# poja/Cattus

Measured on AMD Instinct MI355X. Metric: MCTS node-evals/sec (chess 20x256 net, batch 256), higher is better.
Workload: dtype f16x2

## Files before the change

### cattus_amd/csrc/evaluator.hip

```cpp
#include <hip/hip_runtime.h>

#include <algorithm>
#include <atomic>
#include <chrono>
#include <condition_variable>
#include <cmath>
#include <cstdarg>
#include <cstdio>
#include <cstdlib>
#include <cstring>
#include <deque>
#include <functional>
#include <map>
#include <memory>
#include <mutex>
#include <new>
#include <shared_mutex>
#include <string>
#include <thread>
#include <vector>

#include <dlfcn.h>

#include "../../include/cattus_hip.h"
// ... 112 lines not shown
            return CATTUS_OK;
        }
        hipError_t e = hipMalloc(&p, bytes ? bytes : 16);
        if (e != hipSuccess) return fail(CATTUS_E_NOMEM, "hipMalloc(%zu) failed: %s", bytes, hipGetErrorString(e));
        return CATTUS_OK;
    }
    int upload(const void* src, size_t bytes, DevArena* arena = nullptr) {
        int rc = alloc(bytes, arena);
        if (rc) return rc;
        HIP_TRY(hipMemcpy(p, src, bytes, hipMemcpyHostToDevice));
        return CATTUS_OK;
    }
    template <typename T>
    T* as() const {
        return reinterpret_cast<T*>(p);
    }
};

struct PinnedBuf {
    void* p = nullptr;
    ~PinnedBuf() {
        if (p) (void)hipHostFree(p);
    }
    int alloc(size_t bytes) {
        hipError_t e = hipHostMalloc(&p, bytes ? bytes : 16, hipHostMallocDefault);
        if (e != hipSuccess) return fail(CATTUS_E_NOMEM, "hipHostMalloc(%zu) failed: %s", bytes, hipGetErrorString(e));
        return CATTUS_OK;
    }
    template <typename T>
    T* as() const {
        return reinterpret_cast<T*>(p);
    }
};

std::shared_mutex g_pin_mu;
std::map<const char*, size_t> g_pinned;
struct Roctx {
    int (*push)(const char*) = nullptr;
    int (*pop)() = nullptr;
    Roctx() {
        const char* on = getenv("CATTUS_ROCTX");
        if (!on || on[0] != '1') return;
        for (const char* name : {"librocprofiler-sdk-roctx.so", "libroctx64.so"}) {
            if (void* h = dlopen(name, RTLD_NOW | RTLD_GLOBAL)) {
                push = reinterpret_cast<int (*)(const char*)>(dlsym(h, "roctxRangePushA"));
                pop = reinterpret_cast<int (*)()>(dlsym(h, "roctxRangePop"));
                if (push && pop) return;
                push = nullptr, pop = nullptr;
// ... 28 lines not shown
}

struct ConvLayer {
    DevBuf w, b;
    DevBuf wf;
    DevBuf wu, bw;
    uint32_t cin = 0;
};

struct ServerBatch {
    uint64_t seq = 0;
    uint32_t count = 0, collected = 0;
    bool sealed = false, running = false, done = false;
    int status = CATTUS_OK;
    std::string error;
    std::chrono::steady_clock::time_point t0;
    std::vector<uint64_t> planes;
    std::vector<float> policy, value;
    std::vector<uint8_t> taken;
};

constexpr int NLANES = CATTUS_HIP_LANES;

struct Lane {
    hipStream_t stream = nullptr;
    hipEvent_t done = nullptr;
    DevBuf d_planes, x0, a, t, y, hv, h1, d_policy, d_value;
    DevBuf d_legal_idx, d_legal_cnt, d_probs;
    uint32_t legal_stride = 0;
    PinnedBuf h_planes, h_policy, h_value;
    DevBuf tower_layers, tower_ready;
    PinnedBuf h_tower_err;
    uint32_t tower_nlayers = 0;
    std::mutex mu;
    ~Lane() {
        if (done) (void)hipEventDestroy(done);
        if (stream) (void)hipStreamDestroy(stream);
    }
};

}

struct cattus_eval {
    DevArena arena;
    cattus_net_desc d{};
    cattus_eval_config cfg{};
    bool tuned = false;
    bool simple = false;
    DevBuf d1w, d1b, d2w, d2b, svw, svb, spw, spb;
    bool wait_spin = true;
    Act act = Act::F32;
    uint32_t hw = 0, bpad = 0, cpad0 = 0;
    uint32_t slots = 64;
    uint32_t fpad = 0;
    bool tower64 = false;
    bool resident_tower = true;
    DevBuf t64_layers;
    bool tower64s = false;
    DevBuf t64s_bias;
    bool t64s_fuse_heads = true;
// ... 6 lines not shown
    bool wino_persist = true;
    std::atomic<bool> persist_ok{true};
    uint32_t persist_spin = 1u << 18;
    uint32_t cus = 0;
    bool wino_inplace = true;
    bool split_wfrag = true;
    bool stream_shift_on = true;
    int stream_shift = 0;
    ConvOpts conv_opts;
    DevBuf d_saturated;
    bool t64_layer_steps = true;
    int device = 0;

    ConvLayer stem;
    std::vector<std::unique_ptr<ConvLayer>> c1, c2;
    DevBuf head_w, head_b, w1t, b1, w2, b2, wpt, bp;
    uint32_t kvp = 0, kpp = 0;

    Lane lanes[NLANES];
    std::atomic<unsigned> lane_rr{0};

    std::mutex stat_mu;
    cattus_stats stats{};
    uint64_t stats_tower_fallbacks = 0;

    std::mutex srv_mu;
    std::condition_variable srv_cv, done_cv;
    std::deque<std::unique_ptr<ServerBatch>> batches;
    uint64_t next_seq = 1;
    bool flush_req = false, stop = false;
    std::thread servers[NLANES];

    ~cattus_eval() {
        {
            std::lock_guard<std::mutex> lk(srv_mu);
            stop = true;
        }
        srv_cv.notify_all();
        done_cv.notify_all();
        for (auto& t : servers)
            if (t.joinable()) t.join();
    }
};

namespace {

size_t blob_floats(const cattus_net_desc& d) {
    const size_t hw = (size_t)d.board * d.board, F = d.filters;
    if (F == 0) {
        const size_t K = (size_t)d.planes * hw;
        return 2 * (K * K + K) + K + 1 + (size_t)d.moves * K + d.moves;
    }
    size_t n = F * d.planes * 9 + 4 * F;
    n += (size_t)d.blocks * (2 * F * F * 9 + 6 * F);
    n += (size_t)d.vhc * F + 2 * (size_t)d.vhc + (size_t)FC_HIDDEN * d.vhc * hw + FC_HIDDEN + FC_HIDDEN + 1;
    n += (size_t)d.phc * F + 2 * (size_t)d.phc + (size_t)d.moves * d.phc * hw + d.moves;
    return n;
}

bool wino_shape_ok(const cattus_eval* e, uint32_t cin, uint32_t cout) {
    return e->wino_k4 ? wino4_supported(e->bpad, cin, cout, e->d.board) : wino_supported(e->bpad, cin, cout, e->d.board);
}

std::mutex g_chain_mu;
hipEvent_t g_chain[64] = {};
int chain_persistent_launch(int device, hipStream_t st, const std::function<void()>& launch) {
    std::lock_guard<std::mutex> lk(g_chain_mu);
    hipEvent_t& ev = g_chain[device & 63];
    if (!ev) {
        HIP_TRY(hipEventCreateWithFlags(&ev, hipEventDisableTiming));
    } else {
        HIP_TRY(hipStreamWaitEvent(st, ev, 0));
    }
    launch();
    HIP_TRY(hipEventRecord(ev, st));
    return CATTUS_OK;
}

int upload_conv(cattus_eval* e, ConvLayer& L, const Folded& f, uint32_t cout, uint32_t cin, uint32_t cout_pad, uint32_t cin_pad) {
    int rc;
    if (!e->tuned) {
        L.cin = cin;
        if ((rc = L.b.upload(f.b.data(), cout * sizeof(float)))) return rc;
        return L.w.upload(f.w.data(), f.w.size() * sizeof(float));
    }
    L.cin = cin_pad;
    if (e->act == Act::F16S) {
        std::vector<float> b((size_t)2 * cout_pad, 0.0f);
        memcpy(b.data(), f.b.data(), cout * sizeof(float));
        std::vector<_Float16> w((size_t)9 * cout_pad * 2 * cin_pad, (_Float16)0.0f);
        for (uint32_t co = 0; co < cout_pad; co++) {
            float m = 0.0f;
            if (co < cout)
                for (uint32_t t = 0; t < 9; t++)
                    for (uint32_t ci = 0; ci < cin; ci++) m = std::max(m, fabsf(f.w[((size_t)t * cout + co) * cin + ci]));
            int sh = 0;
            if (m > 0.0f && std::isfinite(m)) sh = std::min(100, std::max(-100, 10 - ilogbf(m)));
            b[cout_pad + co] = ldexpf(1.0f, -sh);
            if (co >= cout) continue;
// ... 270 lines not shown
        HIP_TRY(hipEventCreateWithFlags(&L.done, hipEventBlockingSync | hipEventDisableTiming));
        if ((rc = L.d_planes.alloc(B * d.planes * e->cfg.plane_words * 8))) return rc;
        if ((rc = L.x0.alloc(bp_ * slots * e->cpad0 * esz))) return rc;
        if ((rc = L.a.alloc(bp_ * slots * FA * esz, &e->arena))) return rc;
        if ((rc = L.t.alloc(bp_ * slots * FA * esz, &e->arena))) return rc;
        if ((rc = L.y.alloc(bp_ * slots * FA * esz, e->wino_inplace ? nullptr : &e->arena))) return rc;
        const size_t hv_bytes = (size_t)(e->tuned ? (bp_ + 31) / 32 * 32 : bp_) * (e->kvp + e->kpp) * hesz;
        if ((rc = L.hv.alloc(hv_bytes))) return rc;
        HIP_TRY(hipMemset(L.hv.p, 0, hv_bytes));
        if ((rc = L.h1.alloc(bp_ * FC_HIDDEN * 4))) return rc;
        if ((rc = L.d_policy.alloc(B * d.moves * 4))) return rc;
        if ((rc = L.d_value.alloc(B * 4))) return rc;
        if ((rc = L.h_planes.alloc(B * d.planes * e->cfg.plane_words * 8))) return rc;
        if ((rc = L.h_policy.alloc(B * d.moves * 4))) return rc;
        if ((rc = L.h_value.alloc(B * 4))) return rc;
        if (e->tuned && e->act == Act::F16S && e->wino_k4 && e->wino_persist && e->wino_inplace && d.blocks > 0 && e->c1[0]->wu.p) {
            std::vector<Wino4TowerLayer> tl;
            for (uint32_t i = 0; i < d.blocks; i++) {
                tl.push_back(Wino4TowerLayer{L.a.as<float>(), e->c1[i]->wu.p, e->c1[i]->bw.as<float>(), nullptr, L.t.as<float>()});
                tl.push_back(Wino4TowerLayer{L.t.as<float>(), e->c2[i]->wu.p, e->c2[i]->bw.as<float>(), L.a.as<float>(), L.a.as<float>()});
            }
            L.tower_nlayers = (uint32_t)tl.size();
            if ((rc = L.tower_layers.upload(tl.data(), tl.size() * sizeof(Wino4TowerLayer)))) return rc;
            if ((rc = L.tower_ready.alloc(64 + (size_t)tl.size() * (bp_ / 4) * 4))) return rc;
            if ((rc = L.h_tower_err.alloc(4))) return rc;
            *L.h_tower_err.as<unsigned>() = 0;
        }
    }
    return CATTUS_OK;
}

struct TowerTimer {
    std::vector<hipEvent_t> ev;
    size_t used = 0;
};

int enqueue_forward(cattus_eval* e, Lane& L, const uint64_t* d_planes, uint32_t n, float* d_policy, float* d_value,
                    hipStream_t st, TowerTimer* tt = nullptr) {
    const cattus_net_desc& d = e->d;
    const uint32_t F = d.filters, hw = e->hw, S = d.board, w64 = e->cfg.plane_words;
    auto ev = [&](bool stop) -> hipEvent_t {
        if (!tt || tt->used >= tt->ev.size()) return nullptr;
        (void)stop;
        return tt->ev[tt->used++];
    };
    void *a = L.a.p, *t = L.t.p, *y = L.y.p;
    uint32_t nb = n;
    if (e->simple) {
        const uint32_t K = d.planes * hw;
// ... 36 lines not shown
            launch_tower64_split(ta, nb * e->slots, e->t64s_depth, st, s0, s1);
        } else {
            const bool fused_stem = d.planes <= 32 && e->cpad0 == (uint32_t)act_kc(e->act) && !e->pack_separately;
            const StemInput stem_in{d_planes, n, d.planes, w64};
            if (!fused_stem) launch_pack_planes_nhwc(e->act, d_planes, n, nb, d.planes, w64, S, e->cpad0, L.x0.p, st);
            hipEvent_t s0 = ev(false), s1 = ev(true);
            const int last_flags = act_f16_family(e->act) ? CONV_OUT_F32 : 0;
            const bool wfrag = e->act == Act::F16S && e->split_wfrag;
            const int wflag = wfrag ? CONV_W_FRAG : 0;
            auto wptr = [&](const ConvLayer& c) { return wfrag ? c.wf.p : c.w.p; };
            launch_conv3x3_mfma(e->act, L.x0.p, wptr(e->stem), e->stem.b.as<float>(), nullptr, a, nb, e->cpad0, FP, S, st, s0, s1,
                                fused_stem ? &stem_in : nullptr,
                                wflag | (d.blocks == 0 ? last_flags : e->act == Act::F16S && e->c1[0]->wu.p ? CONV_OUT_F32 | CONV_WINO_IN : 0), e->conv_opts);
            const bool wino = d.blocks > 0 && e->c1[0]->wu.p != nullptr;
            auto conv = [&](const ConvLayer& c, const void* in, const void* res, void* out, int lflags) {
                hipEvent_t s0 = ev(false), s1 = ev(true);
                if (wino && e->wino_k8) launch_conv3x3_wino8((const float*)in, c.wu.p, c.bw.as<float>(), (const float*)res, (float*)out, nb, FP, FP, st, s0, s1, e->conv_opts.saturated);
                else if (wino && e->wino_k4) launch_conv3x3_wino4((const float*)in, c.wu.p, c.bw.as<float>(), (const float*)res, (float*)out, nb, FP, FP, st, s0, s1, e->conv_opts.saturated);
                else if (wino) launch_conv3x3_wino((const float*)in, c.wu.p, c.bw.as<float>(), (const float*)res, (float*)out, nb, FP, FP, st, s0, s1, e->conv_opts.saturated);
                else launch_conv3x3_mfma(e->act, in, wptr(c), c.b.as<float>(), res, out, nb, FP, FP, S, st, s0, s1, nullptr, wflag | lflags, e->conv_opts);
            };
            if (wino && !e->wino_k8 && L.tower_nlayers && e->persist_ok.load(std::memory_order_relaxed) && wino4_tower_fits(nb, FP, e->cus)) {
                hipEvent_t s0 = ev(false), s1 = ev(true);
                unsigned* const tower_err = L.tower_ready.as<unsigned>();
                HIP_TRY(hipMemsetAsync(L.tower_ready.p, 0, 64 + (size_t)L.tower_nlayers * (nb / 4) * 4, st));
                int crc = chain_persistent_launch(e->device, st, [&] {
                    launch_tower_wino4(L.tower_layers.as<Wino4TowerLayer>(), L.tower_nlayers, tower_err + 16, tower_err,
                                       e->conv_opts.saturated, nb, FP, e->persist_spin, e->cus, st, s0, s1);
                });
                if (crc) return crc;
                HIP_TRY(hipMemcpyAsync(L.h_tower_err.p, tower_err, 4, hipMemcpyDeviceToHost, st));
            } else
            for (uint32_t i = 0; i < d.blocks; i++) {
                conv(*e->c1[i], a, nullptr, t, 0);
                if (wino && e->wino_inplace) {
                    conv(*e->c2[i], t, a, a, 0);
                    continue;
                }
                conv(*e->c2[i], t, a, y, i + 1 == d.blocks ? last_flags : 0);
                std::swap(a, y);
            }
        }
    } else {
        launch_planes_to_tensor_nchw(d_planes, n, d.planes, w64, S, n, L.x0.as<float>(), st);
        hipEvent_t s0 = ev(false), s1 = ev(true);
        launch_conv3x3_generic(L.x0.as<float>(), e->stem.w.as<float>(), e->stem.b.as<float>(), nullptr, (float*)a, n,
                               d.planes, F, S, st, s0, s1);
        for (uint32_t i = 0; i < d.blocks; i++) {
            s0 = ev(false), s1 = ev(true);
            launch_conv3x3_generic((float*)a, e->c1[i]->w.as<float>(), e->c1[i]->b.as<float>(), nullptr, (float*)t, n, F,
                                   F, S, st, s0, s1);
            s0 = ev(false), s1 = ev(true);
            launch_conv3x3_generic((float*)t, e->c2[i]->w.as<float>(), e->c2[i]->b.as<float>(), (float*)a, (float*)y, n,
                                   F, F, S, st, s0, s1);
// ... 4 lines not shown
    if (e->tuned) {
        HeadsMfma hd{};
        hd.conv_w = e->head_w.p, hd.conv_b = e->head_b.as<float>(), hd.hv = L.hv.p;
        hd.w1 = e->w1t.p, hd.b1 = e->b1.as<float>(), hd.h1 = L.h1.as<float>();
        hd.wp = e->wpt.p, hd.bp = e->bp.as<float>(), hd.policy = d_policy;
        hd.hw = hw, hd.vhc = d.vhc, hd.phc = d.phc, hd.kvp = e->kvp, hd.kpp = e->kpp, hd.M = d.moves;
        hd.w2 = e->w2.as<float>(), hd.b2 = e->b2.as<float>(), hd.value = d_value;
        hd.slots = e->slots;
        hd.hv_leaves = (e->bpad + 31) / 32 * 32;
        launch_heads_mfma(head_act(e->act), e->tower64 || (e->tower64s && e->t64s_fuse_heads) ? nullptr : a, n, e->fpad, hd, st);
    } else {
        TowerView tv;
        tv.x = a, tv.act = Act::F32, tv.sb = F * hw, tv.sk = hw, tv.sp = 1;
        launch_head_conv1x1(tv, e->head_w.as<float>(), e->head_b.as<float>(), n, F, d.vhc + d.phc, hw, L.hv.as<float>(), st);
        launch_value_fc1(L.hv.as<float>(), kv + kp, e->w1t.as<float>(), e->b1.as<float>(), n, kv, L.h1.as<float>(), st);
        launch_value_fc2_tanh(L.h1.as<float>(), e->w2.as<float>(), e->b2.as<float>(), n, d_value, st);
        launch_policy_fc(L.hv.as<float>(), kv + kp, kv, e->wpt.as<float>(), e->bp.as<float>(), n, kp, d.moves, d_policy, st);
    }
    hipError_t err = hipGetLastError();
    if (err != hipSuccess) return fail(CATTUS_E_DEVICE, "kernel launch failed: %s", hipGetErrorString(err));
    return CATTUS_OK;
}

void account(cattus_eval* e, uint32_t n, double seconds) {
    std::lock_guard<std::mutex> lk(e->stat_mu);
    cattus_stats& s = e->stats;
    s.run_seconds_ema = 0.01 * s.run_seconds_ema + 0.99 * seconds;
    s.run_seconds_total += seconds;
    s.batches += 1;
    s.positions += n;
    if (n == e->cfg.max_batch) s.full_batches += 1;
}

struct LegalArgs {
    const uint16_t* idx;
    const uint16_t* cnt;
    uint32_t stride;
    float* probs;
};

int eval_host(cattus_eval* e, const uint64_t* planes, uint32_t n, float* policy, float* value, const LegalArgs* lg = nullptr) {
    const cattus_net_desc& d = e->d;
    std::unique_lock<std::mutex> lk;
    Lane* lane = nullptr;
    for (Lane& cand : e->lanes) {
        std::unique_lock<std::mutex> tl(cand.mu, std::try_to_lock);
// ... 34 lines not shown
                                     lg->stride, n, L.d_probs.as<float>(), L.stream))
                return fail(CATTUS_E_INVALID, "legal stride %u exceeds 1024", lg->stride);
            HIP_TRY(hipMemcpyAsync(lg->probs, L.d_probs.p, (size_t)n * lg->stride * 4, hipMemcpyDeviceToHost, L.stream));
        } else {
            HIP_TRY(hipMemcpyAsync(direct ? (void*)policy : L.h_policy.p, L.d_policy.p, (size_t)n * d.moves * 4, hipMemcpyDeviceToHost, L.stream));
        }
        HIP_TRY(hipMemcpyAsync(direct ? (void*)value : L.h_value.p, L.d_value.p, (size_t)n * 4, hipMemcpyDeviceToHost, L.stream));
        return CATTUS_OK;
    };
    auto run_batch = [&]() -> int {
        int rc = enqueue_forward(e, L, L.d_planes.as<uint64_t>(), n, L.d_policy.as<float>(), L.d_value.as<float>(), L.stream);
        if (rc) return rc;
        if ((rc = copy_out())) return rc;
        if (e->wait_spin) {
            HIP_TRY(hipStreamSynchronize(L.stream));
        } else {
            HIP_TRY(hipEventRecord(L.done, L.stream));
            HIP_TRY(hipEventSynchronize(L.done));
        }
        return CATTUS_OK;
    };
    int rc = run_batch();
    if (rc) return rc;
    if (L.h_tower_err.p && *L.h_tower_err.as<volatile unsigned>() != 0) {
        *L.h_tower_err.as<volatile unsigned>() = 0;
        e->persist_ok.store(false, std::memory_order_relaxed);
        {
            std::lock_guard<std::mutex> sl(e->stat_mu);
            e->stats_tower_fallbacks += 1;
        }
        if ((rc = run_batch())) return rc;
    }
    if (!direct) {
        if (!lg) memcpy(policy, L.h_policy.p, (size_t)n * d.moves * 4);
        memcpy(value, L.h_value.p, (size_t)n * 4);
    }
    account(e, n, std::chrono::duration<double>(std::chrono::steady_clock::now() - t0).count());
    return CATTUS_OK;
}

ServerBatch* new_batch(cattus_eval* e) {
    auto b = std::make_unique<ServerBatch>();
    b->seq = e->next_seq++;
    b->planes.resize((size_t)e->cfg.max_batch * e->d.planes * e->cfg.plane_words);
    e->batches.push_back(std::move(b));
    return e->batches.back().get();
}

void server_loop(cattus_eval* e) {
    std::unique_lock<std::mutex> lk(e->srv_mu);
    for (;;) {
        ServerBatch* run = nullptr;
        for (auto& b : e->batches)
// ... 20 lines not shown
            e->srv_cv.wait(lk);
            continue;
        }
        run->running = true;
        const uint32_t n = run->count;
        run->policy.resize((size_t)n * e->d.moves);
        run->value.resize(n);
        run->taken.assign(n, 0);
        lk.unlock();
        const int rc = eval_host(e, run->planes.data(), n, run->policy.data(), run->value.data());
        std::string err = rc ? g_last_error : std::string();
        lk.lock();
        run->status = rc;
        run->error = err;
        run->done = true;
        e->done_cv.notify_all();
    }
}

}


CATTUS_API const char* cattus_hip_last_error(void) { return g_last_error.c_str(); }
CATTUS_API const char* cattus_hip_version(void) { return "cattus_hip 0.2 (gfx950)"; }
CATTUS_API const char* cattus_hip_runtime_note(void) { return g_runtime_note.c_str(); }

CATTUS_API const char* cattus_hip_tower_kernel(const cattus_eval* e) {
    if (!e) return "";
    if (e->simple) return "policy_fc_kernel";
    if (!e->tuned) return "conv3x3_generic_kernel";
    if (e->tower64) return "tower64_lds_kernel";
    if (e->tower64s) return "tower64_split_kernel";
    if (e->act == Act::F16S) return e->d.blocks > 0 && e->c1[0]->wu.p ? (e->wino_k8 ? "conv3x3_wino8_kernel" : e->wino_k4 ? (e->lanes[0].tower_nlayers && e->persist_ok.load() && wino4_tower_fits(e->bpad, e->fpad, e->cus) ? "tower_wino4_kernel" : "conv3x3_wino4_kernel") : "conv3x3_wino_kernel") : e->split_wfrag ? "conv3x3_splitw_kernel" : "conv3x3_split_kernel";
    return "conv3x3_mfma_v2_kernel";
}

CATTUS_API int cattus_hip_stream_shift(const cattus_eval* e) { return e ? e->stream_shift : 0; }

namespace {

struct Switches {
    std::map<std::string, std::string> kv;
    int parse(const char* text) {
        if (!text) return CATTUS_OK;
        static const char* const known[] = {"CATTUS_CONV_CB", "CATTUS_CONV_PBW", "CATTUS_FUSED_STEM", "CATTUS_T64_CH", "CATTUS_T64_LS", "CATTUS_SPLIT_W",
                                            "CATTUS_T64S_HEADS", "CATTUS_T64S_SHAPE", "CATTUS_TOWER64", "CATTUS_FORCE_GENERIC", "CATTUS_WINO_INPLACE",
                                            "CATTUS_ARENA", "CATTUS_WINO_KERNEL", "CATTUS_WINO_PERSIST", "CATTUS_WINO_SPIN", "CATTUS_STREAM_SHIFT"};
// ... 207 lines not shown
    for (uint32_t i = 0; i < n; i++) {
        if (legal_count[i] > legal_stride) return fail(CATTUS_E_INVALID, "leaf %u: %u legal moves > stride %u", i, legal_count[i], legal_stride);
        for (uint32_t k = 0; k < legal_count[i]; k++)
            if (legal_idx[(size_t)i * legal_stride + k] >= e->d.moves)
                return fail(CATTUS_E_INVALID, "leaf %u: policy index %u >= %u", i, legal_idx[(size_t)i * legal_stride + k], e->d.moves);
    }
    const LegalArgs lg{legal_idx, legal_count, legal_stride, probs};
    return eval_host(e, planes, n, nullptr, value, &lg);
}

CATTUS_API int cattus_hip_eval_device(cattus_eval* e, const uint64_t* d_planes, uint32_t n, float* d_policy, float* d_value,
                                      void* stream) {
    return cattus_hip_eval_device_lane(e, 0, d_planes, n, d_policy, d_value, stream);
}

CATTUS_API int cattus_hip_eval_device_lane(cattus_eval* e, uint32_t lane, const uint64_t* d_planes, uint32_t n, float* d_policy,
                                           float* d_value, void* stream) {
    if (!e || !d_planes || !d_policy || !d_value) return fail(CATTUS_E_INVALID, "NULL argument");
    if (n < 1 || n > e->cfg.max_batch) return fail(CATTUS_E_INVALID, "invalid sample len %u, 1..=%u", n, e->cfg.max_batch);
    if (lane >= NLANES) return fail(CATTUS_E_INVALID, "lane %u out of range (%d lanes)", lane, NLANES);
    Lane& L = e->lanes[lane];
    std::lock_guard<std::mutex> lk(L.mu);
    HIP_TRY(hipSetDevice(e->device));
    if (L.h_tower_err.p && *L.h_tower_err.as<volatile unsigned>() != 0) {
        *L.h_tower_err.as<volatile unsigned>() = 0;
        e->persist_ok.store(false, std::memory_order_relaxed);
        return fail(CATTUS_E_DEVICE, "an earlier batch on lane %u ran the tower as one launch and a hand-off wait in it gave up (the device was shared): that batch's "
                                     "outputs are invalid; this evaluator uses the per-layer launches from now on", lane);
    }
    hipStream_t st = (hipStream_t)stream;
    int rc = enqueue_forward(e, L, d_planes, n, d_policy, d_value, st);
    if (rc) return rc;
    std::lock_guard<std::mutex> sl(e->stat_mu);
    e->stats.batches += 1;
    e->stats.positions += n;
    if (n == e->cfg.max_batch) e->stats.full_batches += 1;
    return CATTUS_OK;
}

CATTUS_API int cattus_hip_lane_stream(cattus_eval* e, uint32_t lane, void** stream) {
    if (!e || !stream) return fail(CATTUS_E_INVALID, "NULL argument");
    if (lane >= NLANES) return fail(CATTUS_E_INVALID, "lane %u out of range (%d lanes)", lane, NLANES);
    *stream = (void*)e->lanes[lane].stream;
    return CATTUS_OK;
}

CATTUS_API int cattus_hip_submit(cattus_eval* e, const uint64_t* planes_one, uint64_t* ticket) {
    if (!e || !planes_one || !ticket) return fail(CATTUS_E_INVALID, "NULL argument");
    const size_t words = (size_t)e->d.planes * e->cfg.plane_words;
    std::unique_lock<std::mutex> lk(e->srv_mu);
    if (e->stop) return fail(CATTUS_E_STATE, "evaluator is shutting down");
// ... 111 lines not shown
CATTUS_API int cattus_hip_time_tower(cattus_eval* e, uint32_t n, uint32_t reps, float* avg_launch_us, uint32_t* launches) {
    if (!e || !avg_launch_us || !launches) return fail(CATTUS_E_INVALID, "NULL argument");
    if (n < 1 || n > e->cfg.max_batch || reps < 1) return fail(CATTUS_E_INVALID, "bad n/reps");
    if (e->simple) return fail(CATTUS_E_UNSUPPORTED, "a SimpleTwoHeadedModel has no conv tower to time");
    Lane& L = e->lanes[0];
    std::lock_guard<std::mutex> lk(L.mu);
    HIP_TRY(hipSetDevice(e->device));
    const uint32_t per_fwd = e->tower64 || e->tower64s ? 1 : 1 + 2 * e->d.blocks;
    TowerTimer tt;
    tt.ev.resize((size_t)2 * per_fwd);
    for (auto& ev : tt.ev) HIP_TRY(hipEventCreate(&ev));
    HIP_TRY(hipMemsetAsync(L.d_planes.p, 0x5a, (size_t)n * e->d.planes * e->cfg.plane_words * 8, L.stream));
    double total_ms = 0;
    int rc = CATTUS_OK;
    for (uint32_t rep = 0; rep < reps + 1 && rc == CATTUS_OK; rep++) {
        tt.used = 0;
        rc = enqueue_forward(e, L, L.d_planes.as<uint64_t>(), n, L.d_policy.as<float>(), L.d_value.as<float>(), L.stream, &tt);
        if (rc) break;
        hipError_t err = hipStreamSynchronize(L.stream);
        if (err != hipSuccess) {
            rc = fail(CATTUS_E_DEVICE, "hipStreamSynchronize: %s", hipGetErrorString(err));
            break;
        }
        if (rep == 0) continue;
        for (size_t i = 0; i + 1 < tt.used; i += 2) {
            float ms = 0;
            (void)hipEventElapsedTime(&ms, tt.ev[i], tt.ev[i + 1]);
            total_ms += ms;
        }
    }
    for (auto& ev : tt.ev) (void)hipEventDestroy(ev);
    if (rc) return rc;
    *launches = per_fwd;
    *avg_launch_us = (float)(total_ms * 1000.0 / ((double)reps * per_fwd));
    return CATTUS_OK;
}

CATTUS_API int cattus_hip_mfma_sustained(cattus_eval* e, double seconds, double* tflops) {
    if (!e || !tflops) return fail(CATTUS_E_INVALID, "NULL argument");
    if (!(seconds > 0) || seconds > 30) return fail(CATTUS_E_INVALID, "seconds out of range");
    Lane& L = e->lanes[0];
    std::lock_guard<std::mutex> lk(L.mu);
    HIP_TRY(hipSetDevice(e->device));
    hipDeviceProp_t prop;
    HIP_TRY(hipGetDeviceProperties(&prop, e->device));
    const int cus = prop.multiProcessorCount;
// ... 60 lines not shown
```

### cattus_amd/csrc/kernels.h

```cpp
#pragma once
#include <hip/hip_runtime.h>
#include <stdint.h>

namespace cattus {

inline uint32_t tower_slots(uint32_t S) { return S <= 8 ? 64u : 128u; }
constexpr int ROWS_PER_WG = 256;
constexpr int COUT_PER_WG = 64;

enum class Act : int { F32 = 0, BF16 = 1, F16S = 2, F16 = 3 };

inline bool act_two_bytes(Act a) { return a == Act::BF16 || a == Act::F16; }
inline int act_bytes(Act a) { return act_two_bytes(a) ? 2 : 4; }
inline int act_kc(Act a) { return act_two_bytes(a) ? 64 : 32; }
inline Act head_act(Act a) { return a == Act::BF16 ? Act::BF16 : Act::F32; }
inline bool act_f16_family(Act a) { return a == Act::F16S || a == Act::F16; }

hipError_t prepare_device();

void launch_pack_planes_nhwc(Act act, const uint64_t* planes, uint32_t n, uint32_t bpad, uint32_t C,
                             uint32_t w64, uint32_t S, uint32_t cpad, void* out, hipStream_t st);
void launch_planes_to_tensor_nchw(const uint64_t* planes, uint32_t n, uint32_t C, uint32_t w64, uint32_t S,
                                  uint32_t batch, float* out, hipStream_t st);

// ... 24 lines not shown
    const uint32_t nst = cin_pad / 16 * 16, stage = (ci >> 4) * 16 + f, lane = ((ci >> 3) & 1) * 32 + (co & 31);
    return ((((size_t)(co >> 5) * nst + stage) * 2 + part) * 64 + lane) * 8 + (ci & 7);
}
void launch_conv3x3_wino(const float* in, const void* wu, const float* bias, const float* res, float* out, uint32_t bpad, uint32_t cin,
                         uint32_t cout, hipStream_t st, hipEvent_t ev_start, hipEvent_t ev_stop, unsigned* sat);
hipError_t prepare_wino();

bool wino4_supported(uint32_t bpad, uint32_t cin, uint32_t cout, uint32_t S);
void launch_conv3x3_wino4(const float* in, const void* wu, const float* bias, const float* res, float* out, uint32_t bpad, uint32_t cin,
                          uint32_t cout, hipStream_t st, hipEvent_t ev_start, hipEvent_t ev_stop, unsigned* sat);
hipError_t prepare_wino4();
bool wino8_supported(uint32_t bpad, uint32_t cin, uint32_t cout, uint32_t S);
void launch_conv3x3_wino8(const float* in, const void* wu, const float* bias, const float* res, float* out, uint32_t bpad, uint32_t cin,
                          uint32_t cout, hipStream_t st, hipEvent_t ev_start, hipEvent_t ev_stop, unsigned* sat);
hipError_t prepare_wino8();
struct Wino4TowerLayer {
    const float* in;
    const void* wu;
    const float* bias;
    const float* res;
    float* out;
};
bool wino4_tower_fits(uint32_t bpad, uint32_t filters, uint32_t cus);
void launch_tower_wino4(const Wino4TowerLayer* d_layers, uint32_t nlayers, unsigned* ready, unsigned* err, unsigned* sat, uint32_t bpad, uint32_t filters,
                        uint32_t spin_budget, uint32_t cus, hipStream_t st, hipEvent_t ev_start, hipEvent_t ev_stop);

double launch_mfma_sustain(Act act, int cus, int iters, float* out, hipStream_t st);

struct Tower64Layer {
    const void* w;
    const float* bias;
    int res;
    int pad_;
};
struct Tower64Args {
    const uint64_t* planes;
    const Tower64Layer* layers;
    void* out;
    uint32_t n, C, w64, S, nlayers;
    const void* head_w;
    const float* head_b;
    void* hv;
    uint32_t hv_pol, kvp, kpp, vhc, ocn;
};
void launch_tower64(const Tower64Args& args, uint32_t rows, int ch, bool layer_steps, hipStream_t st,
                    hipEvent_t ev_start = nullptr, hipEvent_t ev_stop = nullptr);

// ... 65 lines not shown
```

### cattus_amd/csrc/kernels_wino4.hip

```cpp
#include "kernels.h"
#include "device_common.h"

#include <hip/hip_ext.h>

namespace cattus {

constexpr int W4_TROW = 8 * SP;
constexpr int W4_IMG = 9472;
constexpr int W4_ZAREA = 512;
constexpr int W4_IMGZ = W4_IMG + W4_ZAREA;
constexpr int W4_DBUF = 8 * W4_IMGZ;
constexpr int W4_LDS_LOOP = 2 * W4_DBUF;
constexpr int W4_LDS_Z = 4 * 2 * 64 * 256;
constexpr int W4_LDS_TOTAL = W4_LDS_Z > W4_LDS_LOOP ? W4_LDS_Z : W4_LDS_LOOP;
static_assert(W4_IMG % 256 == 0 && W4_IMGZ % 256 == 0 && W4_DBUF % 256 == 0, "the zero area keeps a read's banks only if everything is 256-B aligned");
static_assert(W4_IMG >= 8 * W4_TROW + 16 && W4_ZAREA >= 256 + 128 && W4_LDS_LOOP <= 160 * 1024, "image / zero area / LDS sizes");

typedef __attribute__((ext_vector_type(2))) _Float16 w4_f16x2;

template <int V>
using w4_int = std::integral_constant<int, V>;

#ifdef CATTUS_STAMPS
__device__ unsigned long long g_stamps_w4[1024 * 4 * 10];
// ... 88 lines not shown
                if (ya < 0) asm("v_fma_f32 %0, %1, -1.0, 0" : "=v"(t[e]) : "v"(regs[yb][e]));
                else if (fq == 1) asm("v_fma_f32 %0, %1, 1.0, %2" : "=v"(t[e]) : "v"(regs[yb][e]), "v"(regs[ya][e]));
                else asm("v_fma_f32 %0, %1, -1.0, %2" : "=v"(t[e]) : "v"(regs[yb][e]), "v"(regs[ya][e]));
            }
        }
        typedef __attribute__((address_space(3))) u32x4 w4_lu32x4;
        *(w4_lu32x4*)(uintptr_t)(target + (uint32_t)(fq * 2 * W4_IMGZ + ty * W4_TROW)) = t;
    };
    for (int i = tid; i < 16 * (W4_ZAREA / 16); i += 256)
        reinterpret_cast<f32x4*>(smem + (i / (W4_ZAREA / 16)) * W4_IMGZ + W4_IMG)[i % (W4_ZAREA / 16)] = f32x4{0.f, 0.f, 0.f, 0.f};
    u32x4 first[W4_NP], pend[W4_NP];
    const char* wks = wb0;
    load_ustage(ring[0], wks, 0);
    load_ustage(ring[1], wks, 1);
    if (PERSIST && sync.wait_word) {
        if (tid == 0) {
            unsigned budget = sync.spin_budget, seen = 0, bad = 0;
            for (;;) {
                asm volatile("global_load_dword %0, %1, off sc1\n\ts_waitcnt vmcnt(0)" : "=v"(seen) : "v"(sync.wait_word) : "memory");
                if (seen >= sync.wait_target) break;
                if ((budget & 63) == 0) asm volatile("global_load_dword %0, %1, off sc1\n\ts_waitcnt vmcnt(0)" : "=v"(bad) : "v"(sync.err) : "memory");
                if (bad != 0 || --budget == 0) {
                    atomicExch(sync.err, 1u);
                    break;
                }
                __builtin_amdgcn_s_sleep(8);
            }
        }
        asm volatile("s_barrier" ::: "memory");
    }
    W4_STAMP(8);
    load_chunk(first, 0);
    load_chunk(pend, 1);
    load_ustage(ring[2], wks, 2);

    const int n = lane & 31, hh = lane >> 5;
    const int b2 = n >> 4, ty = (n >> 2) & 3, tx = n & 3;
    uint32_t cur[3];
    {
        const int tbase = (b2 * 4 + ty) * W4_TROW + (2 * tx - 1) * SP + b2 * 16 + hh * 32;
        const int tdelta = tbase - W4_IMG;
        const int mc0 = tx != 0 ? -1 : 255, mc3 = tx != 3 ? -1 : 255;
        const uint32_t img = lds0 + (uint32_t)(q * 2 * W4_IMGZ + W4_IMG);
        cur[0] = img + (uint32_t)(tdelta & mc0);
        cur[1] = img + (uint32_t)(tdelta + SP);
        cur[2] = img + (uint32_t)(((tdelta + 3 * SP) & mc3));
// ... 230 lines not shown
        asm volatile("s_barrier" ::: "memory");
        if (tid == 0) __hip_atomic_fetch_add(sync.done_word, 1u, __ATOMIC_RELAXED, __HIP_MEMORY_SCOPE_AGENT);
    }
#ifdef CATTUS_STAMPS
    W4_STAMP(5);
    W4_STAMP_RT(7);
    if (lane == 0 && blockIdx.x < 1024) {
#pragma unroll
        for (int i = 0; i < 10; i++) g_stamps_w4[((size_t)blockIdx.x * 4 + q) * 10 + i] = st_[i];
    }
#endif
}

template <bool HAS_RES>
__global__ void __launch_bounds__(256, 1)
    conv3x3_wino4_kernel(const float* __restrict__ in, const _Float16* __restrict__ wu, const float* __restrict__ bias,
                         const float* res, float* out, unsigned* __restrict__ sat, int cin, int cout) {
    extern __shared__ __attribute__((aligned(16))) char smem[];
    const W4Sync none{};
    w4_layer<HAS_RES ? 1 : 0, false>(in, wu, bias, res, out, sat, cin, cout, smem, none, (int)blockIdx.x, (int)gridDim.x);
}

__global__ void __launch_bounds__(256, 1)
    tower_wino4_kernel(const Wino4TowerLayer* __restrict__ layers, int nlayers, unsigned* ready, unsigned* err, unsigned* __restrict__ sat, int filters,
                       unsigned spin_budget, int tiles) {
    extern __shared__ __attribute__((aligned(16))) char smem[];
    const int ncg = filters >> 6, ngroups = tiles / ncg;
    auto group_of = [&](int wg) {
        int logical = wg;
        if ((tiles & 7) == 0) logical = (wg & 7) * (tiles >> 3) + (wg >> 3);
        return logical / ncg;
    };
    auto sync_of = [&](int layer, int group) {
        W4Sync sync;
        sync.wait_word = layer > 0 ? ready + (size_t)(layer - 1) * ngroups + group : nullptr;
        sync.done_word = ready + (size_t)layer * ngroups + group;
        sync.err = err, sync.wait_target = (unsigned)ncg, sync.spin_budget = spin_budget;
        return sync;
    };
    for (int layer = 0; layer + 1 < nlayers; layer += 2) {
        const Wino4TowerLayer A = layers[layer];
        for (int wg = blockIdx.x; wg < tiles; wg += gridDim.x)
            w4_layer<0, true>(A.in, reinterpret_cast<const _Float16*>(A.wu), A.bias, nullptr, A.out, sat, filters, filters, smem, sync_of(layer, group_of(wg)), wg, tiles);
        const Wino4TowerLayer B = layers[layer + 1];
        for (int wg = blockIdx.x; wg < tiles; wg += gridDim.x)
            w4_layer<1, true>(B.in, reinterpret_cast<const _Float16*>(B.wu), B.bias, B.res, B.out, sat, filters, filters, smem, sync_of(layer + 1, group_of(wg)), wg, tiles);
    }
}

bool wino4_supported(uint32_t bpad, uint32_t cin, uint32_t cout, uint32_t S) {
    return S == 8 && cin >= 128 && cin % 32 == 0 && cout >= 128 && cout % 64 == 0 && bpad % 4 == 0;
}

void launch_conv3x3_wino4(const float* in, const void* wu, const float* bias, const float* res, float* out, uint32_t bpad, uint32_t cin,
                          uint32_t cout, hipStream_t st, hipEvent_t ev_start, hipEvent_t ev_stop, unsigned* sat) {
    typedef _Float16 H;
    const dim3 grid((bpad / 4) * (cout / 64));
    if (res)
        hipExtLaunchKernelGGL((conv3x3_wino4_kernel<true>), grid, dim3(256), W4_LDS_TOTAL, st, ev_start, ev_stop, 0, in, (const H*)wu, bias, res, out,
                              sat, (int)cin, (int)cout);
    else
        hipExtLaunchKernelGGL((conv3x3_wino4_kernel<false>), grid, dim3(256), W4_LDS_TOTAL, st, ev_start, ev_stop, 0, in, (const H*)wu, bias, res, out,
                              sat, (int)cin, (int)cout);
}

static uint32_t tower_grid(uint32_t tiles, uint32_t cus) { return tiles <= cus ? tiles : cus & ~7u; }

bool wino4_tower_fits(uint32_t bpad, uint32_t filters, uint32_t cus) {
    const uint32_t tiles = (bpad / 4) * (filters / 64);
    return tiles <= cus || (cus >= 8 && tiles % 8 == 0);
}

void launch_tower_wino4(const Wino4TowerLayer* d_layers, uint32_t nlayers, unsigned* ready, unsigned* err, unsigned* sat, uint32_t bpad, uint32_t filters,
                        uint32_t spin_budget, uint32_t cus, hipStream_t st, hipEvent_t ev_start, hipEvent_t ev_stop) {
    const uint32_t tiles = (bpad / 4) * (filters / 64);
    hipExtLaunchKernelGGL(tower_wino4_kernel, dim3(tower_grid(tiles, cus)), dim3(256), W4_LDS_TOTAL, st, ev_start, ev_stop, 0, d_layers, (int)nlayers, ready, err,
                          sat, (int)filters, spin_budget, (int)tiles);
}

#ifdef CATTUS_STAMPS
extern "C" __attribute__((visibility("default"))) int cattus_hip_debug_stamps_w4(unsigned long long* out, size_t n) {
    return (int)hipMemcpyFromSymbol(out, HIP_SYMBOL(g_stamps_w4), n * sizeof(unsigned long long));
}
#endif

hipError_t prepare_wino4() {
    hipError_t err = hipFuncSetAttribute(reinterpret_cast<const void*>(&conv3x3_wino4_kernel<true>), hipFuncAttributeMaxDynamicSharedMemorySize, W4_LDS_TOTAL);
    const hipError_t e2 = hipFuncSetAttribute(reinterpret_cast<const void*>(&conv3x3_wino4_kernel<false>), hipFuncAttributeMaxDynamicSharedMemorySize, W4_LDS_TOTAL);
    const hipError_t e3 = hipFuncSetAttribute(reinterpret_cast<const void*>(&tower_wino4_kernel), hipFuncAttributeMaxDynamicSharedMemorySize, W4_LDS_TOTAL);
    return err != hipSuccess ? err : e2 != hipSuccess ? e2 : e3;
}

}
```

### cattus_amd/evaluator.py

```python

from __future__ import annotations

import ctypes as C
from pathlib import Path

import numpy as np

from .weights import NetDesc, parse_header

import os

_PKG = Path(__file__).resolve().parent
LIB_PATH = Path(os.environ.get("CATTUS_HIP_LIB", _PKG / "libcattus_hip.so"))

DTYPE_F32, DTYPE_BF16, DTYPE_F16X2, DTYPE_F16 = 0, 1, 2, 3
_DTYPES = {"f32": DTYPE_F32, "bf16": DTYPE_BF16, "f16x2": DTYPE_F16X2, "f16": DTYPE_F16}

ABI_SYMBOLS = [
    "cattus_hip_create",
    "cattus_hip_destroy",
    "cattus_hip_desc",
    "cattus_hip_eval",
    "cattus_hip_eval_device",
    "cattus_hip_eval_device_lane",
# ... 31 lines not shown
        ("device", C.c_int32),
        ("max_batch", C.c_uint32),
        ("plane_words", C.c_uint32),
        ("dtype", C.c_uint32),
        ("flush_us", C.c_uint32),
        ("tower_form", C.c_uint32),
    ]


TOWER_FORMS = {"auto": 0, "direct": 1, "winograd": 2}
DIAG_SWITCHES = ("CATTUS_CONV_CB", "CATTUS_CONV_PBW", "CATTUS_FUSED_STEM", "CATTUS_T64_CH", "CATTUS_T64_LS", "CATTUS_SPLIT_W", "CATTUS_T64S_HEADS",
                 "CATTUS_T64S_SHAPE", "CATTUS_TOWER64", "CATTUS_FORCE_GENERIC", "CATTUS_WINO_INPLACE", "CATTUS_ARENA", "CATTUS_WINO_KERNEL",
                 "CATTUS_WINO_PERSIST", "CATTUS_WINO_SPIN", "CATTUS_STREAM_SHIFT")


class Stats(C.Structure):
    _fields_ = [
        ("batches", C.c_uint64),
        ("positions", C.c_uint64),
        ("full_batches", C.c_uint64),
        ("run_seconds_ema", C.c_double),
        ("run_seconds_total", C.c_double),
        ("saturated", C.c_uint64),
    ]


class NetDescC(C.Structure):
    _fields_ = [(n, C.c_uint32) for n in ("planes", "board", "moves", "blocks", "filters", "vhc", "phc", "fc_hidden")]


_lib = None


def load_library():
    global _lib
    if _lib is not None:
        return _lib
    if not LIB_PATH.exists():
        raise FileNotFoundError(
            f"{LIB_PATH} is missing: build it with `python -m cattus_amd.build` "
            "(there is no CPU fallback for the leaf evaluator)"
        )
    L = C.CDLL(str(LIB_PATH))
    u64p, f32p = C.POINTER(C.c_uint64), C.POINTER(C.c_float)
    vp = C.c_void_p
    L.cattus_hip_create.argtypes = [vp, C.c_size_t, C.POINTER(EvalConfig), C.POINTER(vp)]
# ... 190 lines not shown
```

### include/cattus_hip.h

```cpp
#ifndef CATTUS_HIP_H
#define CATTUS_HIP_H

#include <stddef.h>
#include <stdint.h>

#ifdef __cplusplus
extern "C" {
#endif

typedef struct cattus_eval cattus_eval;

typedef enum cattus_status {
    CATTUS_OK = 0,
    CATTUS_E_INVALID = -1,
    CATTUS_E_UNSUPPORTED = -2,
    CATTUS_E_DEVICE = -3,
    CATTUS_E_NOMEM = -4,
    CATTUS_E_STATE = -5,
} cattus_status;

typedef enum cattus_dtype {
    CATTUS_DTYPE_F32 = 0,
    CATTUS_DTYPE_BF16 = 1,
    CATTUS_DTYPE_F16X2 = 2,
// ... 3 lines not shown
typedef enum cattus_tower_form {
    CATTUS_TOWER_AUTO = 0,
    CATTUS_TOWER_DIRECT = 1,
    CATTUS_TOWER_WINOGRAD = 2,
} cattus_tower_form;

typedef struct cattus_eval_config {
    uint32_t struct_size;
    int32_t device;
    uint32_t max_batch;
    uint32_t plane_words;
    uint32_t dtype;
    uint32_t flush_us;
    uint32_t tower_form;
} cattus_eval_config;

typedef struct cattus_stats {
    uint64_t batches;
    uint64_t positions;
    uint64_t full_batches;
    double run_seconds_ema;
    double run_seconds_total;
    uint64_t saturated;
} cattus_stats;

typedef struct cattus_net_desc {
    uint32_t planes, board, moves, blocks, filters, vhc, phc, fc_hidden;
} cattus_net_desc;

int cattus_hip_create(const void* weights, size_t nbytes, const cattus_eval_config* cfg, cattus_eval** out);
void cattus_hip_destroy(cattus_eval* e);
int cattus_hip_desc(const cattus_eval* e, cattus_net_desc* out);

int cattus_hip_eval(cattus_eval* e, const uint64_t* planes, uint32_t n, float* policy, float* value);

int cattus_hip_eval_legal(cattus_eval* e, const uint64_t* planes, uint32_t n, const uint16_t* legal_idx,
                          const uint16_t* legal_count, uint32_t legal_stride, float* probs, float* value);

int cattus_hip_eval_device(cattus_eval* e, const uint64_t* d_planes, uint32_t n, float* d_policy,
                           float* d_value, void* stream);

#ifndef CATTUS_HIP_LANES
#define CATTUS_HIP_LANES 2
#endif
int cattus_hip_eval_device_lane(cattus_eval* e, uint32_t lane, const uint64_t* d_planes, uint32_t n,
                                float* d_policy, float* d_value, void* stream);
// ... 32 lines not shown
```

### integration/rust/hip.rs

```rust

use std::ffi::{c_char, c_void, CStr};
use std::path::Path;

#[derive(Clone, Copy, Debug, PartialEq, Eq, serde::Deserialize)]
#[serde(rename_all = "lowercase")]
pub enum HipDtype {
    F32 = 0,
    Bf16 = 1,
    F16x2 = 2,
    F16 = 3,
}

#[repr(C)]
struct CattusEvalConfig {
    struct_size: u32,
    device: i32,
    max_batch: u32,
    plane_words: u32,
    dtype: u32,
    flush_us: u32,
    tower_form: u32,
}

#[repr(C)]
#[derive(Default, Debug, Clone, Copy)]
pub struct CattusStats {
    pub batches: u64,
    pub positions: u64,
    pub full_batches: u64,
    pub run_seconds_ema: f64,
    pub run_seconds_total: f64,
    pub saturated: u64,
}

#[repr(C)]
struct CattusEval {
    _private: [u8; 0],
}

extern "C" {
    fn cattus_hip_create(weights: *const c_void, nbytes: usize, cfg: *const CattusEvalConfig, out: *mut *mut CattusEval) -> i32;
    fn cattus_hip_destroy(e: *mut CattusEval);
    fn cattus_hip_apply(e: *mut CattusEval, planes: *const u64, n: u32, policy: *mut f32, value: *mut f32) -> i32;
    fn cattus_hip_eval(e: *mut CattusEval, planes: *const u64, n: u32, policy: *mut f32, value: *mut f32) -> i32;
    fn cattus_hip_flush(e: *mut CattusEval) -> i32;
    fn cattus_hip_stats(e: *mut CattusEval, out: *mut CattusStats) -> i32;
    fn cattus_hip_last_error() -> *const c_char;
}

fn check(rc: i32) {
    if rc != 0 {
        let msg = unsafe { CStr::from_ptr(cattus_hip_last_error()) }.to_string_lossy().into_owned();
        panic!("cattus_hip: {msg} ({rc})");
    }
}
// ... 59 lines not shown
```

Measured before the change: 219,100.

## Double-buffer tower ready flags and drop per-batch memset and error copy

Replaces the per-batch hipMemsetAsync of the persistent tower's hand-off flags with two alternating flag sets. The kernel itself clears the other set at its end, so each launch starts on a set zeroed by the previous one. The error flag is now written by the device straight into mapped coherent host memory, which removes the D2H memcpy after each tower launch. It also skips the cross-stream event wait when the same stream launches again. Together these remove extra stream operations and a small copy per batch. In exchange the fallback path gets more complex: it relies on system-scope stores and a full device sync to recover.

```diff
diff --git a/cattus_amd/csrc/evaluator.hip b/cattus_amd/csrc/evaluator.hip
--- a/cattus_amd/csrc/evaluator.hip
+++ b/cattus_amd/csrc/evaluator.hip
@@ -158,8 +158,8 @@
     ~PinnedBuf() {
         if (p) (void)hipHostFree(p);
     }
-    int alloc(size_t bytes) {
-        hipError_t e = hipHostMalloc(&p, bytes ? bytes : 16, hipHostMallocDefault);
+    int alloc(size_t bytes, unsigned flags = hipHostMallocDefault) {
+        hipError_t e = hipHostMalloc(&p, bytes ? bytes : 16, flags);
         if (e != hipSuccess) return fail(CATTUS_E_NOMEM, "hipHostMalloc(%zu) failed: %s", bytes, hipGetErrorString(e));
         return CATTUS_OK;
     }
@@ -234,6 +234,8 @@
 
 constexpr int NLANES = CATTUS_HIP_LANES;
 
+void chain_forget_stream(hipStream_t st);
+
 struct Lane {
     hipStream_t stream = nullptr;
     hipEvent_t done = nullptr;
@@ -243,11 +245,12 @@
     PinnedBuf h_planes, h_policy, h_value;
     DevBuf tower_layers, tower_ready;
     PinnedBuf h_tower_err;
-    uint32_t tower_nlayers = 0;
+    uint32_t tower_nlayers = 0, tower_set_words = 0;
+    uint32_t tower_launches = 0;
     std::mutex mu;
     ~Lane() {
         if (done) (void)hipEventDestroy(done);
-        if (stream) (void)hipStreamDestroy(stream);
+        if (stream) chain_forget_stream(stream), (void)hipStreamDestroy(stream);
     }
 };
 
@@ -300,7 +303,6 @@
 
     std::mutex stat_mu;
     cattus_stats stats{};
-    uint64_t stats_tower_fallbacks = 0;
 
     std::mutex srv_mu;
     std::condition_variable srv_cv, done_cv;
@@ -342,17 +344,25 @@
 
 std::mutex g_chain_mu;
 hipEvent_t g_chain[64] = {};
+hipStream_t g_chain_stream[64] = {};
 int chain_persistent_launch(int device, hipStream_t st, const std::function<void()>& launch) {
     std::lock_guard<std::mutex> lk(g_chain_mu);
     hipEvent_t& ev = g_chain[device & 63];
+    hipStream_t& last = g_chain_stream[device & 63];
     if (!ev) {
         HIP_TRY(hipEventCreateWithFlags(&ev, hipEventDisableTiming));
-    } else {
+    } else if (last != st) {
         HIP_TRY(hipStreamWaitEvent(st, ev, 0));
     }
     launch();
     HIP_TRY(hipEventRecord(ev, st));
-    return CATTUS_OK;
+    last = st;
+    return CATTUS_OK;
+}
+void chain_forget_stream(hipStream_t st) {
+    std::lock_guard<std::mutex> lk(g_chain_mu);
+    for (int i = 0; i < 64; i++)
+        if (g_chain[i] && g_chain_stream[i] == st) g_chain_stream[i] = reinterpret_cast<hipStream_t>(~(uintptr_t)0);
 }
 
 int upload_conv(cattus_eval* e, ConvLayer& L, const Folded& f, uint32_t cout, uint32_t cin, uint32_t cout_pad, uint32_t cin_pad) {
@@ -669,9 +679,15 @@
             }
             L.tower_nlayers = (uint32_t)tl.size();
             if ((rc = L.tower_layers.upload(tl.data(), tl.size() * sizeof(Wino4TowerLayer)))) return rc;
-            if ((rc = L.tower_ready.alloc(64 + (size_t)tl.size() * (bp_ / 4) * 4))) return rc;
-            if ((rc = L.h_tower_err.alloc(4))) return rc;
-            *L.h_tower_err.as<unsigned>() = 0;
+            L.tower_set_words = (uint32_t)((tl.size() * (bp_ / 4) + 3) / 4 * 4);
+            const size_t ready_bytes = 64 + (size_t)2 * L.tower_set_words * 4;
+            if ((rc = L.tower_ready.alloc(ready_bytes))) return rc;
+            HIP_TRY(hipMemset(L.tower_ready.p, 0, ready_bytes));
+            if ((rc = L.h_tower_err.alloc(64, hipHostMallocMapped | hipHostMallocCoherent))) return rc;
+            *L.h_tower_err.as<volatile unsigned>() = 0;
+            void* err_host = nullptr;
+            HIP_TRY(hipHostGetDevicePointer(&err_host, L.h_tower_err.p, 0));
+            HIP_TRY(hipMemcpy((char*)L.tower_ready.p + 8, &err_host, sizeof err_host, hipMemcpyHostToDevice));
         }
     }
     return CATTUS_OK;
@@ -754,14 +770,12 @@
             };
             if (wino && !e->wino_k8 && L.tower_nlayers && e->persist_ok.load(std::memory_order_relaxed) && wino4_tower_fits(nb, FP, e->cus)) {
                 hipEvent_t s0 = ev(false), s1 = ev(true);
-                unsigned* const tower_err = L.tower_ready.as<unsigned>();
-                HIP_TRY(hipMemsetAsync(L.tower_ready.p, 0, 64 + (size_t)L.tower_nlayers * (nb / 4) * 4, st));
+                const Wino4TowerSync ts{L.tower_ready.as<unsigned>(), L.tower_set_words, L.tower_launches & 1};
                 int crc = chain_persistent_launch(e->device, st, [&] {
-                    launch_tower_wino4(L.tower_layers.as<Wino4TowerLayer>(), L.tower_nlayers, tower_err + 16, tower_err,
-                                       e->conv_opts.saturated, nb, FP, e->persist_spin, e->cus, st, s0, s1);
+                    launch_tower_wino4(L.tower_layers.as<Wino4TowerLayer>(), L.tower_nlayers, ts, e->conv_opts.saturated, nb, FP, e->persist_spin, e->cus, st, s0, s1);
                 });
                 if (crc) return crc;
-                HIP_TRY(hipMemcpyAsync(L.h_tower_err.p, tower_err, 4, hipMemcpyDeviceToHost, st));
+                L.tower_launches++;
             } else
             for (uint32_t i = 0; i < d.blocks; i++) {
                 conv(*e->c1[i], a, nullptr, t, 0);
@@ -812,6 +826,19 @@
     return CATTUS_OK;
 }
 
+bool tower_gave_up(const Lane& L) { return L.h_tower_err.p && *L.h_tower_err.as<volatile unsigned>() != 0; }
+
+int tower_fall_back(cattus_eval* e, Lane& L) {
+    e->persist_ok.store(false, std::memory_order_relaxed);
+    HIP_TRY(hipDeviceSynchronize());
+    HIP_TRY(hipMemset(L.tower_ready.p, 0, 4));
+    HIP_TRY(hipMemset((char*)L.tower_ready.p + 64, 0, (size_t)2 * L.tower_set_words * 4));
+    *L.h_tower_err.as<volatile unsigned>() = 0;
+    std::lock_guard<std::mutex> sl(e->stat_mu);
+    e->stats.tower_fallbacks += 1;
+    return CATTUS_OK;
+}
+
 void account(cattus_eval* e, uint32_t n, double seconds) {
     std::lock_guard<std::mutex> lk(e->stat_mu);
     cattus_stats& s = e->stats;
@@ -892,13 +919,8 @@
     };
     int rc = run_batch();
     if (rc) return rc;
-    if (L.h_tower_err.p && *L.h_tower_err.as<volatile unsigned>() != 0) {
-        *L.h_tower_err.as<volatile unsigned>() = 0;
-        e->persist_ok.store(false, std::memory_order_relaxed);
-        {
-            std::lock_guard<std::mutex> sl(e->stat_mu);
-            e->stats_tower_fallbacks += 1;
-        }
+    if (tower_gave_up(L)) {
+        if ((rc = tower_fall_back(e, L))) return rc;
         if ((rc = run_batch())) return rc;
     }
     if (!direct) {
@@ -965,7 +987,7 @@
 
 
 CATTUS_API const char* cattus_hip_last_error(void) { return g_last_error.c_str(); }
-CATTUS_API const char* cattus_hip_version(void) { return "cattus_hip 0.2 (gfx950)"; }
+CATTUS_API const char* cattus_hip_version(void) { return "cattus_hip 0.3 (gfx950)"; }
 CATTUS_API const char* cattus_hip_runtime_note(void) { return g_runtime_note.c_str(); }
 
 CATTUS_API const char* cattus_hip_tower_kernel(const cattus_eval* e) {
@@ -1219,11 +1241,11 @@
     Lane& L = e->lanes[lane];
     std::lock_guard<std::mutex> lk(L.mu);
     HIP_TRY(hipSetDevice(e->device));
-    if (L.h_tower_err.p && *L.h_tower_err.as<volatile unsigned>() != 0) {
-        *L.h_tower_err.as<volatile unsigned>() = 0;
-        e->persist_ok.store(false, std::memory_order_relaxed);
-        return fail(CATTUS_E_DEVICE, "an earlier batch on lane %u ran the tower as one launch and a hand-off wait in it gave up (the device was shared): that batch's "
-                                     "outputs are invalid; this evaluator uses the per-layer launches from now on", lane);
+    if (tower_gave_up(L)) {
+        int frc = tower_fall_back(e, L);
+        if (frc) return frc;
+        return fail(CATTUS_E_DEVICE, "an earlier batch on lane %u ran the tower as one launch and a hand-off wait in it gave up (the device was shared): the outputs of that "
+                                     "batch and of those enqueued behind it are invalid; this evaluator uses the per-layer launches from now on", lane);
     }
     hipStream_t st = (hipStream_t)stream;
     int rc = enqueue_forward(e, L, d_planes, n, d_policy, d_value, st);
@@ -1381,6 +1403,12 @@
             rc = fail(CATTUS_E_DEVICE, "hipStreamSynchronize: %s", hipGetErrorString(err));
             break;
         }
+        if (tower_gave_up(L)) {
+            if (!(rc = tower_fall_back(e, L)))
+                rc = fail(CATTUS_E_DEVICE, "a hand-off wait of the one-launch tower gave up during the timing pass (the device was shared): nothing was timed; "
+                                           "this evaluator uses the per-layer launches from now on");
+            break;
+        }
         if (rep == 0) continue;
         for (size_t i = 0; i + 1 < tt.used; i += 2) {
             float ms = 0;
diff --git a/cattus_amd/csrc/kernels.h b/cattus_amd/csrc/kernels.h
--- a/cattus_amd/csrc/kernels.h
+++ b/cattus_amd/csrc/kernels.h
@@ -70,7 +70,12 @@
     float* out;
 };
 bool wino4_tower_fits(uint32_t bpad, uint32_t filters, uint32_t cus);
-void launch_tower_wino4(const Wino4TowerLayer* d_layers, uint32_t nlayers, unsigned* ready, unsigned* err, unsigned* sat, uint32_t bpad, uint32_t filters,
+struct Wino4TowerSync {
+    unsigned* words;
+    uint32_t set_words;
+    uint32_t set;
+};
+void launch_tower_wino4(const Wino4TowerLayer* d_layers, uint32_t nlayers, const Wino4TowerSync& sync, unsigned* sat, uint32_t bpad, uint32_t filters,
                         uint32_t spin_budget, uint32_t cus, hipStream_t st, hipEvent_t ev_start, hipEvent_t ev_stop);
 
 double launch_mfma_sustain(Act act, int cus, int iters, float* out, hipStream_t st);
diff --git a/cattus_amd/csrc/kernels_wino4.hip b/cattus_amd/csrc/kernels_wino4.hip
--- a/cattus_amd/csrc/kernels_wino4.hip
+++ b/cattus_amd/csrc/kernels_wino4.hip
@@ -134,6 +134,7 @@
                 if ((budget & 63) == 0) asm volatile("global_load_dword %0, %1, off sc1\n\ts_waitcnt vmcnt(0)" : "=v"(bad) : "v"(sync.err) : "memory");
                 if (bad != 0 || --budget == 0) {
                     atomicExch(sync.err, 1u);
+                    __hip_atomic_store(*reinterpret_cast<unsigned* const*>(sync.err + 2), 1u, __ATOMIC_RELAXED, __HIP_MEMORY_SCOPE_SYSTEM);
                     break;
                 }
                 __builtin_amdgcn_s_sleep(8);
@@ -410,8 +411,8 @@
 }
 
 __global__ void __launch_bounds__(256, 1)
-    tower_wino4_kernel(const Wino4TowerLayer* __restrict__ layers, int nlayers, unsigned* ready, unsigned* err, unsigned* __restrict__ sat, int filters,
-                       unsigned spin_budget, int tiles) {
+    tower_wino4_kernel(const Wino4TowerLayer* __restrict__ layers, int nlayers, unsigned* words, unsigned* __restrict__ sat, int filters, unsigned spin_budget,
+                       int tiles, unsigned set_words, unsigned set) {
     extern __shared__ __attribute__((aligned(16))) char smem[];
     const int ncg = filters >> 6, ngroups = tiles / ncg;
     auto group_of = [&](int wg) {
@@ -421,9 +422,10 @@
     };
     auto sync_of = [&](int layer, int group) {
         W4Sync sync;
+        unsigned* const ready = words + 16 + set * set_words;
         sync.wait_word = layer > 0 ? ready + (size_t)(layer - 1) * ngroups + group : nullptr;
         sync.done_word = ready + (size_t)layer * ngroups + group;
-        sync.err = err, sync.wait_target = (unsigned)ncg, sync.spin_budget = spin_budget;
+        sync.err = words, sync.wait_target = (unsigned)ncg, sync.spin_budget = spin_budget;
         return sync;
     };
     for (int layer = 0; layer + 1 < nlayers; layer += 2) {
@@ -434,6 +436,8 @@
         for (int wg = blockIdx.x; wg < tiles; wg += gridDim.x)
             w4_layer<1, true>(B.in, reinterpret_cast<const _Float16*>(B.wu), B.bias, B.res, B.out, sat, filters, filters, smem, sync_of(layer + 1, group_of(wg)), wg, tiles);
     }
+    u32x4* const other = reinterpret_cast<u32x4*>(words + 16 + (set ^ 1u) * set_words);
+    for (unsigned i = blockIdx.x * 256 + threadIdx.x; i < set_words / 4; i += gridDim.x * 256) other[i] = u32x4{0u, 0u, 0u, 0u};
 }
 
 bool wino4_supported(uint32_t bpad, uint32_t cin, uint32_t cout, uint32_t S) {
@@ -459,11 +463,11 @@
     return tiles <= cus || (cus >= 8 && tiles % 8 == 0);
 }
 
-void launch_tower_wino4(const Wino4TowerLayer* d_layers, uint32_t nlayers, unsigned* ready, unsigned* err, unsigned* sat, uint32_t bpad, uint32_t filters,
+void launch_tower_wino4(const Wino4TowerLayer* d_layers, uint32_t nlayers, const Wino4TowerSync& sync, unsigned* sat, uint32_t bpad, uint32_t filters,
                         uint32_t spin_budget, uint32_t cus, hipStream_t st, hipEvent_t ev_start, hipEvent_t ev_stop) {
     const uint32_t tiles = (bpad / 4) * (filters / 64);
-    hipExtLaunchKernelGGL(tower_wino4_kernel, dim3(tower_grid(tiles, cus)), dim3(256), W4_LDS_TOTAL, st, ev_start, ev_stop, 0, d_layers, (int)nlayers, ready, err,
-                          sat, (int)filters, spin_budget, (int)tiles);
+    hipExtLaunchKernelGGL(tower_wino4_kernel, dim3(tower_grid(tiles, cus)), dim3(256), W4_LDS_TOTAL, st, ev_start, ev_stop, 0, d_layers, (int)nlayers, sync.words,
+                          sat, (int)filters, spin_budget, (int)tiles, sync.set_words, sync.set);
 }
 
 #ifdef CATTUS_STAMPS
diff --git a/cattus_amd/evaluator.py b/cattus_amd/evaluator.py
--- a/cattus_amd/evaluator.py
+++ b/cattus_amd/evaluator.py
@@ -77,6 +77,7 @@
         ("run_seconds_ema", C.c_double),
         ("run_seconds_total", C.c_double),
         ("saturated", C.c_uint64),
+        ("tower_fallbacks", C.c_uint64),
     ]
 
 
diff --git a/include/cattus_hip.h b/include/cattus_hip.h
--- a/include/cattus_hip.h
+++ b/include/cattus_hip.h
@@ -49,6 +49,7 @@
     double run_seconds_ema;
     double run_seconds_total;
     uint64_t saturated;
+    uint64_t tower_fallbacks;
 } cattus_stats;
 
 typedef struct cattus_net_desc {
diff --git a/integration/rust/hip.rs b/integration/rust/hip.rs
--- a/integration/rust/hip.rs
+++ b/integration/rust/hip.rs
@@ -31,6 +31,7 @@
     pub run_seconds_ema: f64,
     pub run_seconds_total: f64,
     pub saturated: u64,
+    pub tower_fallbacks: u64,
 }
 
 #[repr(C)]
```

Result: no change. 219,900, median of 6 (+0.4%).
